# viniciusvidal2/slam-sensor-fusion

Hardware: AMD Instinct MI355X
Metric: scans_per_s_200k_scan_vs_10M_map (higher is better)
Workload: dtype f32 points / f64 accumulation

## Files before the change

### include/slamfusion.h

```cpp
#ifndef SLAMFUSION_H
#define SLAMFUSION_H
#include <stdint.h>

#ifdef __cplusplus
extern "C" {
#endif

#define SF_VERSION 210

typedef enum {
    SF_OK = 0,
    SF_ERR_INVALID = -1,
    SF_ERR_HIP = -2,
    SF_ERR_NOMEM = -3,
    SF_ERR_STATE = -4,
    SF_ERR_OVERFLOW = -5,
    SF_ERR_COMM = -6
} sf_status;

typedef struct sf_ctx sf_ctx;
typedef struct sf_cloud sf_cloud;
typedef struct sf_map sf_map;
typedef struct sf_icp sf_icp;

// ... 252 lines not shown
int sf_icp_fetch_previous(sf_icp *icp, sf_icp_result *out);
int sf_icp_use_graph(sf_icp *icp, int on);
int sf_icp_graph_counts(sf_icp *icp, int64_t *captures, int64_t *launches);
int sf_icp_set_fused(sf_icp *icp, int on);
int sf_icp_fused_count(sf_icp *icp, int64_t *launches);
int sf_icp_fused_redone(sf_icp *icp, int64_t *redone);
int sf_icp_test_inject_barrier_timeout(sf_icp *icp);
#define SF_ORDER_AUTO 0
#define SF_ORDER_AS_GIVEN 1
#define SF_ORDER_CELL 2
int sf_icp_set_query_order(sf_icp *icp, int order);
int sf_icp_set_nn_reuse(sf_icp *icp, int on);
int sf_icp_set_wide_scan_points(sf_icp *icp, int64_t points);
int sf_icp_set_pipeline(sf_icp *icp, int on);
int sf_icp_set_tile_search(sf_icp *icp, int mode);
int sf_icp_tile_info(sf_icp *icp, int64_t out[12]);
int sf_icp_set_freeze(sf_icp *icp, int on);
int sf_icp_set_freeze_params(sf_icp *icp, float guard_scale, float guard_min, float guard_max, int max_tries, int from_launch);
int sf_icp_freeze_stats(sf_icp *icp, int64_t out[5]);
int sf_icp_set_defer_search(sf_icp *icp, int on);
int sf_icp_defer_stats(sf_icp *icp, int64_t out[2]);
int sf_icp_lookup_launch_stats(sf_icp *icp, int64_t out[4]);
int sf_icp_set_neighbour_research(sf_icp *icp, int from_launch);
int sf_icp_neighbour_stats(sf_icp *icp, int64_t out[3]);
int sf_icp_neighbour_gap_stats(sf_icp *icp, int64_t out[4]);
#define SF_ROBUST_NONE 0
#define SF_ROBUST_HUBER 1
#define SF_ROBUST_CAUCHY 2
#define SF_ROBUST_TUKEY 3
#define SF_ROBUST_GM 4
int sf_icp_set_robust_kernel(sf_icp *icp, int kind, double k);

#define SF_COV_EIG_EPS 1e-12
#define SF_COV_FEW_CORR 1
#define SF_COV_SINGULAR 2
#define SF_COV_DEGENERATE_TRANS 4
#define SF_COV_DEGENERATE_ROT 8
typedef struct {
    double info[36];
    double cov[36];
    double sigma2, sigma2_hat, weight_sum;
    double trans_info[3], trans_dir[9];
    double rot_info[3], rot_dir[9];
    int64_t n_corr;
    int32_t flags;
} sf_icp_covariance;
// ... 218 lines not shown
```

### slam_sensor_fusion_amd/api.py

```python
import atexit
import ctypes as C
import math
import os
import weakref

import numpy as np

_HERE = os.path.dirname(os.path.abspath(__file__))
LIB_PATH = os.path.join(_HERE, "lib", "libslamfusion.so")

SF_ICP_REF_CPP, SF_ICP_O3D_P2P, SF_ICP_P2PLANE = 0, 1, 2
SF_VOXEL_PCL, SF_VOXEL_O3D, SF_VOXEL_PCL64 = 0, 1, 2
SF_FLAG_VOXEL_OVERFLOW = 1
SF_ICP_FLAG_FEW_CORR, SF_ICP_FLAG_SINGULAR, SF_ICP_FLAG_SHARD_STALE, SF_ICP_FLAG_BARRIER_TIMEOUT = 1, 2, 4, 8
PROF_NN, PROF_REDUCE, PROF_COLLECTIVE, PROF_SOLVE, PROF_SHARD_BUILD = 0, 1, 2, 3, 4
SF_ERR_COMM = -6
MODES = {"ref_cpp": SF_ICP_REF_CPP, "o3d_p2p": SF_ICP_O3D_P2P, "p2plane": SF_ICP_P2PLANE}
ROBUST_KINDS = {"none": 0, "huber": 1, "cauchy": 2, "tukey": 3, "gm": 4}


class SlamFusionError(RuntimeError):
    pass


# ... 1515 lines not shown
        code = {False: 0, "off": 0, "auto": 1, True: 2, "always": 2}[on]
        _check(self.lib.sf_icp_set_tile_search(self.h, C.c_int(code)))

    def tile_info(self):
        a = (C.c_int64 * 12)()
        _check(self.lib.sf_icp_tile_info(self.h, a))
        return {"on": bool(a[0]), "cells_per_tile": [a[1], a[2], a[3]], "tiles": [a[4], a[5], a[6]], "searched": a[7], "from_lds": a[8], "left_region": a[9],
                "beyond_ring_1": a[10], "tiles_too_dense": a[11]}

    def set_freeze_params(self, guard_scale=8.0, guard_min=2.0e-5, guard_max=3.0e-4, max_tries=3, from_launch=5):
        _check(self.lib.sf_icp_set_freeze_params(self.h, C.c_float(guard_scale), C.c_float(guard_min), C.c_float(guard_max), C.c_int(max_tries), C.c_int(from_launch)))

    def freeze_stats(self):
        a = (C.c_int64 * 5)()
        _check(self.lib.sf_icp_freeze_stats(self.h, a))
        return {"froze": a[0], "thawed": a[1], "failed": a[2], "active_queries": a[3], "frozen_at_end": a[4]}

    def set_defer_search(self, on=True):
        _check(self.lib.sf_icp_set_defer_search(self.h, C.c_int(int(bool(on)))))

    def set_neighbour_research(self, from_launch=2):
        _check(self.lib.sf_icp_set_neighbour_research(self.h, C.c_int(int(from_launch))))

    def neighbour_stats(self):
        a = (C.c_int64 * 3)()
        _check(self.lib.sf_icp_neighbour_stats(self.h, a))
        return {"served": a[0], "not_served": a[1], "waves_searched": a[2]}

    def neighbour_gap_stats(self):
        a = (C.c_int64 * 4)()
        _check(self.lib.sf_icp_neighbour_gap_stats(self.h, a))
        return {"served": a[0], "not_served": a[1], "waves_searched": a[2], "by_gap": a[3]}

    def defer_stats(self):
        a = (C.c_int64 * 2)()
        _check(self.lib.sf_icp_defer_stats(self.h, a))
        return {"deferred_queries": a[0], "capped_waves": a[1]}

    def lookup_launch_stats(self):
        a = (C.c_int64 * 4)()
        _check(self.lib.sf_icp_lookup_launch_stats(self.h, a))
        return {"launches": a[0], "deferred_queries": a[1], "capped_waves": a[2], "first": a[3]}

    def set_query_order(self, order="auto"):
        _check(self.lib.sf_icp_set_query_order(self.h, C.c_int({"auto": 0, "as_given": 1, "cell": 2}[order])))

# ... 689 lines not shown
```

### slam_sensor_fusion_amd/csrc/sf_icp.hip

```cpp
#include "sf_common.hpp"
#include "sf_nn.hpp"
#include "sf_tile.hpp"
#include "sf_order.hpp"
#include "sf_p2p.hpp"
#include "sf_schedule.hpp"
#include "sf_sort.hpp"

#include <cfloat>
#include <cstdlib>
#include <cmath>
#include <vector>
#include <mutex>
#include <string>
#include <type_traits>

namespace {

constexpr int BLK = 256;
constexpr int NREC_P2P = 17;
constexpr int NREC_PLANE = 30;
constexpr int REC_STRIDE = 32;

struct IcpState {
    double T[16];
// ... 1781 lines not shown
        }
    }
#pragma unroll
    for (int h = 0; h < 2; ++h) {
        double v[16];
#pragma unroll
        for (int k = 0; k < 16; ++k) v[k] = 0.0;
#pragma unroll
        for (int u = 0; u < Q; ++u) {
            const PairTerms t = pair_terms<MODE>(P[u]);
            add_half<MODE>(t, h, v);
        }
        const double t0 = wave_reduce_16(v);
        if ((lane & 3) == 0) stage[wv][16 * h + (lane >> 2)] = t0;
    }
    __syncthreads();
    if (threadIdx.x < NREC) {
        const int c = threadIdx.x;
        double *dst = partials + ((size_t)b * nblocks + bx) * REC_STRIDE;
        dst[c] = ((stage[0][c] + stage[1][c]) + stage[2][c]) + stage[3][c];
    }
}

template <int Q>
__global__ __launch_bounds__(BLK, 2) void k_nn_deferred(SfGrid g, SfWindow w, const float *__restrict__ X0x, const float *__restrict__ X0y, const float *__restrict__ X0z,
                                                                   int n, const IcpState *__restrict__ st, float thr, int nblocks, float4 *__restrict__ qcache, int64_t cache_n,
                                                                   uint32_t *__restrict__ stats, DeferBufs df)
{
    constexpr int MODE = 2;
    constexpr int NW = BLK / 64;
    const int r = (int)blockIdx.x, b = (int)blockIdx.y;
    const IcpState *S = st + b;
    if (S->done) return;
    __shared__ sf::WaveNN nn_ws[NW];
    __shared__ double fstage[NW][32];
    __shared__ uint32_t list[BLK * DF_WCAP];
    __shared__ uint32_t wsum[NW];
    __shared__ uint32_t capped;
    const int wv = threadIdx.x >> 6, lane = threadIdx.x & 63;
    if (threadIdx.x == 0) capped = 0u;
    __syncthreads();
    const int my_rows = r < nblocks ? (nblocks - r + FZ_FEW - 1) / FZ_FEW : 0;
    const int nseg = my_rows * NW;
    double acc = 0.0;
    uint32_t n_listed = 0;
    for (int s0 = 0; s0 < nseg; s0 += BLK) {
        const int sg = s0 + (int)threadIdx.x;
        const int bx = r + (sg / NW) * FZ_FEW;
        const size_t seg = ((size_t)b * nblocks + bx) * NW + (sg % NW);
        uint32_t c = sg < nseg ? (uint32_t)df.cnt[seg] : 0u;
        if (c > (uint32_t)DF_WCAP) {
            atomicAdd(&capped, 1u);
            c = 0u;
        }
        uint32_t incl = c;
#pragma unroll
        for (int off = 1; off < 64; off <<= 1) {
            const uint32_t t = __shfl_up(incl, off, 64);
            if (lane >= off) incl += t;
        }
        if (lane == 63) wsum[wv] = incl;
        __syncthreads();
        uint32_t base = 0, total = 0;
#pragma unroll
        for (int ww = 0; ww < NW; ++ww) {
            if (ww < wv) base += wsum[ww];
            total += wsum[ww];
        }
        const uint32_t start = base + incl - c;
        for (uint32_t i = 0; i < c; ++i) list[start + i] = (uint32_t)bx * (uint32_t)(BLK * Q) + (uint32_t)df.ids[seg * DF_WCAP + i];
        __syncthreads();
        n_listed += total;
        for (uint32_t q0 = 0; q0 < total; q0 += BLK) {
            const uint32_t i = q0 + (uint32_t)threadIdx.x;
            if (q0 + (uint32_t)(wv * 64) < total) {
                const int slot = i < total ? (int)list[i] : n;
                const LanePair A1 = nn_pair<MODE, false, false>(g, w, X0x, X0y, X0z, n, b, S, thr, 0.0f, 0.0f, nullptr, qcache, cache_n, slot, n, &nn_ws[wv], stats, nullptr, false);
#pragma unroll
                for (int h = 0; h < 2; ++h) {
                    double v[16];
#pragma unroll
                    for (int k = 0; k < 16; ++k) v[k] = 0.0;
                    const PairTerms t = pair_terms<MODE>(A1);
                    add_half<MODE>(t, h, v);
                    const double t0 = wave_reduce_16(v);
                    if ((lane & 3) == 0) fstage[wv][16 * h + (lane >> 2)] = t0;
                }
            } else if (lane < 32) {
                fstage[wv][lane] = 0.0;
            }
            __syncthreads();
            if (threadIdx.x < 32) acc += ((fstage[0][threadIdx.x] + fstage[1][threadIdx.x]) + fstage[2][threadIdx.x]) + fstage[3][threadIdx.x];
            __syncthreads();
        }
    }
    if (threadIdx.x < REC_STRIDE) df.part[((size_t)b * FZ_FEW + r) * REC_STRIDE + threadIdx.x] = threadIdx.x < NREC_PLANE ? acc : 0.0;
    __syncthreads();
    if (threadIdx.x == 0) {
        if (n_listed) atomicAdd(&df.stat[0], n_listed);
        if (capped) {
// ... 821 lines not shown

void prof_collect(sf_icp *icp)
{
    for (size_t k = 0; k + 1 < icp->ev_used; k += 2) {
        float ms = 0;
        if (hipEventElapsedTime(&ms, icp->ev[k], icp->ev[k + 1]) != hipSuccess) continue;
        const int kind = k / 2 < icp->ev_kind.size() ? icp->ev_kind[k / 2] : SF_PROF_NN;
        if (kind == SF_PROF_NN) { icp->prof_ms += ms; icp->prof_launches += 1; icp->prof_each.push_back(ms); }
        else if (kind > 0 && kind < SF_PROF_KINDS) icp->prof_phase[kind].push_back(ms);
    }
    icp->ev_used = 0;
}

void schedule_describe(sf_icp *icp, int mode, bool whole)
{
    const SrcSet &ss = icp->src();
    sf::Schedule in;
    in.mode = mode; in.K = icp->prm.num_iters; in.qpl = ss.qpl; in.sharded = icp->shard; in.whole = whole; in.reuse = icp->reuse; in.window = icp->map->window.kind;
    in.robust = robust_on(icp, mode); in.fz_from = icp->fz_from; in.defer = icp->defer != 0; in.table = icp->nbr_active; in.nbr_from = icp->nbr_active ? icp->nbr_from : -1;
    in.lk_min = icp->lk_min; in.tile_on = icp->tile_on;
    in.wanted = icp->freeze == 2 || (icp->freeze == 1 && (icp->shard ? icp->own_total : ss.n * ss.batch) >= FREEZE_AUTO_MIN_QUERIES);
    icp->cur().meta.sched = sf::make_schedule(in);
    icp->cur().meta.lk_waves = (int64_t)ss.batch * ss.nblocks_nn * (BLK / 64);
}

int slab_rows(const sf_icp *icp, bool sharded, bool one_per_lane)
{
    if (sharded) return one_per_lane ? icp->own_nblocks * icp->src().qpl : icp->own_nblocks;
    return one_per_lane ? icp->src().nblocks : icp->src().nblocks_nn;
}

uint32_t *nn_stats_slot(sf_icp *icp)
{
    if (!icp->profiling || !icp->nn_stats.p || icp->nn_stats_used >= sf_icp::NN_STATS_CAP) return nullptr;
    return icp->nn_stats.as<uint32_t>() + NN_STATS_PER * NN_STATS_SHARDS * icp->nn_stats_used++;
}

sf_icp::GraphKey graph_key_now(const sf_icp *icp, int mode)
{
    const Lane &ln = icp->cur(); const SrcSet &ss = icp->src();
    sf_icp::GraphKey k;
    k.batch = ss.batch; k.ordered = (int)icp->ordered; k.sched = ln.meta.sched;
    k.n = (mode == SF_ICP_REF_CPP && ss.batch == 1) ? -ss.n_cap : ss.n;
    k.map = (const void *)icp->map;
    k.map_generation = icp->map->generation;
    if (icp->nbr_active) { k.nbr_stamp = icp->map->nbr_stamp; k.nbr = icp->map->nbr.p; }
    k.robust_kind = robust_on(icp, mode) ? icp->robust_kind : SF_ROBUST_NONE; k.robust_k = robust_on(icp, mode) ? icp->robust_k : 0.0;
    k.cov_on = icp->cov_on;
    if (icp->cov_on) { const double cp[5] = {icp->cov_arg.sensor_sigma, icp->cov_arg.thr_t, icp->cov_arg.thr_r, icp->cov_arg.infl_t, icp->cov_arg.infl_r}; std::memcpy(k.cov_prm, cp, sizeof(cp)); }
    k.max_corr = icp->prm.max_corr; k.accept = icp->prm.accept; k.eps = icp->prm.eps;
    k.guard_scale = icp->fz_prm.guard_scale; k.guard_min = icp->fz_prm.guard_min; k.guard_max = icp->fz_prm.guard_max; k.max_tries = icp->fz_prm.max_tries;
    const sf::DevBuf *bufs[] = {&ss.X0, &ss.X0r, &ln.X, &ln.Xq, &ln.qcache, &ln.corr, &ln.state, &ln.partials, &icp->d_box, &ss.d_boxes, &ss.n_dev,
                                &icp->map->pts4, &icp->map->nrm4, &icp->map->cell_start, &icp->map->d_window, &ln.fz_state, &ln.fz_part, &ln.fz_cnt, &ln.fz_ids, &ln.fz_all, &ln.df_cnt, &ln.df_ids, &ln.df_part, &ln.df_stat, &ln.tseg, &ln.tile_stats, &ln.cov_part, &ln.cov_out};
    k.epochs = (uint64_t)ss.plane;
    for (const sf::DevBuf *b : bufs) k.epochs = (k.epochs * 1000003ull + b->epoch) * 1000003ull + (uint64_t)(uintptr_t)b->p;
    return k;
}

SfGrid grid_for(const sf_icp *icp)
{
    SfGrid g = icp->map->grid;
    g.nbr = icp->nbr_active ? icp->map->nbr.as<uint4>() : nullptr;
    g.nbr_from = icp->nbr_from;
    return g;
}

int nbr_prepare(sf_icp *icp, int mode)
{
    sf_map *m = icp->map;
    const SrcSet &ss = icp->src();
    icp->nbr_active = false;
// ... 90 lines not shown
{
    Lane &ln = icp->cur();
    FreezeBufs fb;
    fb.fz = on ? ln.fz_state.as<FreezeState>() : nullptr;
    fb.mom_part = ln.fz_part.as<double>();
    fb.act_cnt = ln.fz_cnt.as<uint32_t>();
    fb.act_ids = ln.fz_ids.as<uint16_t>();
    fb.act_all = ln.fz_all.as<uint32_t>();
    fb.df_part = deferred ? ln.df_part.as<double>() : nullptr;
    return fb;
}

DeferBufs defer_bufs(sf_icp *icp)
{
    Lane &ln = icp->cur();
    DeferBufs d;
    d.cnt = ln.df_cnt.as<uint8_t>();
    d.ids = ln.df_ids.as<uint16_t>();
    d.part = ln.df_part.as<double>();
    d.stat = ln.df_stat.as<uint32_t>();
    return d;
}

void launch_nn_deferred(sf_icp *icp, uint32_t *stats)
{
    Lane &ln = icp->cur(); SrcSet &ss = icp->src();
    sf_map *m = icp->map;
    hipLaunchKernelGGL((k_nn_deferred<SF_WIDE_QPL>), dim3((unsigned)FZ_FEW, (unsigned)ss.batch), dim3(BLK), 0, icp->ctx->stream, grid_for(icp), m->window, queries(icp, 0), queries(icp, 1), queries(icp, 2),
                       (int)ss.n, ln.state.as<IcpState>(), o3d_thr(icp), ss.nblocks_nn, ln.qcache.as<float4>(), icp->cache_n, stats, defer_bufs(icp));
}

void launch_nn_red_df(sf_icp *icp, int attempt_from)
{
    Lane &ln = icp->cur(); SrcSet &ss = icp->src();
    sf_map *m = icp->map;
    const int nb = ss.nblocks_nn;
    const dim3 grid((unsigned)((nb + 7) & ~7), (unsigned)ss.batch), blk(BLK);
    ProfScope ps(icp);
    uint32_t *stats = nn_stats_slot(icp);
    hipLaunchKernelGGL((k_nn_red_df<SF_WIDE_QPL>), grid, blk, 0, icp->ctx->stream, grid_for(icp), m->window, queries(icp, 0), queries(icp, 1), queries(icp, 2), (int)ss.n, ln.state.as<IcpState>(),
                       o3d_thr(icp), ln.partials.as<double>(), nb, ln.qcache.as<float4>(), icp->cache_n, stats, defer_bufs(icp), attempt_from);
    launch_nn_deferred(icp, stats);
}

void launch_nn_red_fz(sf_icp *icp, bool sharded, bool few)
{
    Lane &ln = icp->cur(); SrcSet &ss = icp->src();
    sf_map *m = icp->map;
    const int nb = slab_rows(icp, sharded, false);
    const dim3 grid_full((unsigned)((nb + 7) & ~7), (unsigned)ss.batch), grid_few((unsigned)FZ_FEW, (unsigned)ss.batch), blk(BLK);
    ProfScope ps(icp);
    FzArgs A;
    A.X0x = queries(icp, 0); A.X0y = queries(icp, 1); A.X0z = queries(icp, 2);
    A.n = (int)ss.n;
    A.st = ln.state.as<IcpState>();
    A.thr = o3d_thr(icp); A.xlo = icp->xlo; A.xhi = icp->xhi;
    A.partials = ln.partials.as<double>();
    A.nblocks = nb;
    A.own_off = icp->own_off.as<uint32_t>();
    A.qcache = ln.qcache.as<float4>();
    A.cache_n = icp->cache_n;
    A.stats = nn_stats_slot(icp);
    A.fz = ln.fz_state.as<FreezeState>();
    A.mom_part = ln.fz_part.as<double>();
    A.act_cnt = ln.fz_cnt.as<uint32_t>();
    A.act_ids = ln.fz_ids.as<uint16_t>();
    A.act_all = ln.fz_all.as<uint32_t>();
    hipStream_t s = icp->ctx->stream;
    if (few) with_bools([&](auto S) { hipLaunchKernelGGL((k_nn_red_fz_few<SF_WIDE_QPL, S()>), grid_few, blk, 0, s, grid_for(icp), m->window, A); }, sharded);
    else with_bools([&](auto S) { hipLaunchKernelGGL((k_nn_red_fz<SF_WIDE_QPL, S()>), grid_full, blk, 0, s, grid_for(icp), m->window, A); }, sharded);
}

template <int MODE>
void launch_nn(sf_icp *icp, const sf::LaunchStep &step, bool sharded)
{
    if (step.frozen()) launch_nn_red_fz(icp, sharded, step.nn == sf::NN_FROZEN_FEW);
    else if (step.nn == sf::NN_DEFERRING) launch_nn_red_df(icp, step.attempt_from);
    else if (step.nn == sf::NN_TILE_SEARCH) launch_tile_search<MODE>(icp, step.one_per_lane);
    else launch_nn_red<MODE>(icp, sharded, step.one_per_lane);
}

int step_start_pass(sf_icp *icp, int mode)
{
    Lane &ln = icp->cur(); SrcSet &ss = icp->src();
    icp->fz_step = 0;
    schedule_describe(icp, mode, false);
    if (!ln.meta.sched.fz) return SF_OK;
    SF_TRY(freeze_alloc(icp));
    hipLaunchKernelGGL(k_fz_init, dim3(nblk(ss.batch, 64)), dim3(64), 0, icp->ctx->stream, ln.fz_state.as<FreezeState>(), ss.batch, ln.df_stat.as<uint32_t>());
    return SF_OK;
}

int launch_state_init(sf_icp *icp)
{
    Lane &ln = icp->cur();
    hipStream_t s = icp->ctx->stream;
    const int B = icp->src().batch;
    InitArgs args;
    if (B <= INIT_ARGS_MAX) {
        std::memcpy(args.T, icp->inits.data(), sizeof(double) * 16 * (size_t)B);
// ... 536 lines not shown
{
    SF_CHECK(icp && out, SF_ERR_INVALID, "bad arguments");
    for (int i = 0; i < 12; ++i) out[i] = 0;
    out[0] = icp->tile_on ? 1 : 0;
    if (!icp->tile_on) return SF_OK;
    for (int a = 0; a < 3; ++a) { out[1 + a] = icp->tiles.tc[a]; out[4 + a] = icp->tiles.nt[a]; }
    if (icp->cur().tile_stats.p) {
        SF_HIP(hipSetDevice(icp->ctx->device));
        unsigned long long h[TILE_STATS];
        SF_HIP(hipMemcpyAsync(h, icp->cur().tile_stats.p, sizeof(h), hipMemcpyDeviceToHost, icp->ctx->stream));
        SF_HIP(hipStreamSynchronize(icp->ctx->stream));
        for (int i = 0; i < 5; ++i) out[7 + i] = (int64_t)h[i];
    }
    return SF_OK;
}

extern "C" int sf_icp_set_defer_search(sf_icp *icp, int on)
{
    SF_CHECK(icp, SF_ERR_INVALID, "icp is NULL");
    icp->defer = on != 0;
    return SF_OK;
}

extern "C" int sf_icp_set_neighbour_research(sf_icp *icp, int from_launch)
{
    SF_CHECK(icp, SF_ERR_INVALID, "icp is NULL");
    SF_CHECK(from_launch != 0, SF_ERR_INVALID, "from_launch must be at least 1 (the first launch has no cached neighbours), or negative for off");
    icp->nbr_from = from_launch < 0 ? -1 : from_launch;
    icp->lk_min = 0;
    return SF_OK;
}

namespace {
int neighbour_stats(sf_icp *icp, int64_t out[4])
{
    SF_CHECK(icp && out, SF_ERR_INVALID, "bad arguments");
    SF_CHECK(icp->profiling && icp->nn_stats.p, SF_ERR_STATE, "the neighbour statistics are counted in profiled runs (sf_icp_profile_enable)");
    SF_CHECK(icp->nn_stats_used < sf_icp::NN_STATS_CAP, SF_ERR_STATE, "the profiling counters are full (%lld launches since sf_icp_profile_enable): enable profiling again to reset them", (long long)sf_icp::NN_STATS_CAP);
    SF_HIP(hipStreamSynchronize(icp->ctx->stream));
    out[0] = out[1] = out[2] = out[3] = 0;
    const int64_t first = icp->nbr_stats_first, used = icp->nn_stats_used;
    if (used <= first) return SF_OK;
    const size_t per = (size_t)NN_STATS_PER * NN_STATS_SHARDS;
    std::vector<uint32_t> st(per * (size_t)(used - first), 0u);
    SF_HIP(hipMemcpy(st.data(), icp->nn_stats.as<uint32_t>() + per * (size_t)first, sizeof(uint32_t) * st.size(), hipMemcpyDeviceToHost));
    for (size_t i = 0; i < st.size(); i += NN_STATS_PER) { out[0] += st[i + 2]; out[1] += st[i + 3]; out[2] += st[i + 1]; out[3] += st[i + 4]; }
    return SF_OK;
}
}

extern "C" int sf_icp_neighbour_stats(sf_icp *icp, int64_t out[3])
{
// ... 25 lines not shown
    out[0] = out[1] = out[2] = 0;
    out[3] = -1;
    const sf::Schedule &sched = icp->cur().meta.sched;
    if (sched.lookup_launches() <= 0) return SF_OK;
    int64_t df[2];
    SF_TRY(sf_icp_defer_stats(icp, df));
    out[0] = sched.lookup_launches();
    out[1] = df[0];
    out[2] = df[1];
    out[3] = sched.lookup_first;
    return SF_OK;
}

extern "C" int sf_icp_set_freeze(sf_icp *icp, int on)
{
    SF_CHECK(icp, SF_ERR_INVALID, "icp is NULL");
    SF_CHECK(on >= 0 && on <= 2, SF_ERR_INVALID, "sf_icp_set_freeze: 0 (off), 1 (auto) or 2 (always)");
    icp->freeze = on;
    return SF_OK;
}

namespace {
constexpr int FZ_FROM_DEFAULT = 5, FZ_PROBE_EVERY = 32;
void freeze_learn_schedule(sf_icp *icp)
{
    const sf::Schedule &sched = icp->cur().meta.sched;
    if (!icp->fz_from_auto || icp->last_fused || icp->shard || icp->last_mode != SF_ICP_P2PLANE) return;
    const int K = sched.K;
    if (++icp->fz_fetches >= FZ_PROBE_EVERY) { icp->fz_fetches = 0; icp->fz_from = FZ_FROM_DEFAULT; icp->lk_min = 0; return; }
    if (!sched.fz) return;
    if (sched.lookup_launches() > 0 && icp->cur().df_stat.p) {
        uint32_t h[2 + DF_STAT_LAUNCHES];
        if (hipMemcpy(h, icp->cur().df_stat.p, sizeof(h), hipMemcpyDeviceToHost) == hipSuccess) {
            for (int k = sched.lookup_first; k < sched.fz_from && k < DF_STAT_LAUNCHES - 1; ++k)
                if ((int64_t)h[2 + k] * 8 > icp->cur().meta.lk_waves) icp->lk_min = std::max(icp->lk_min, k + 1);
        }
    }
    int latest = -1, never = 0;
    for (int b = 0; b < icp->src().batch; ++b) {
        const IcpState &S = icp->h_state[(size_t)b];
        if (S.froze_launch >= 0) latest = std::max(latest, S.froze_launch);
        else if (S.iterations >= K) never += 1;
    }
    if (latest < 0) icp->fz_from = std::max(FZ_FROM_DEFAULT, K);
    else if (never * 4 <= icp->src().batch) icp->fz_from = std::min(std::max(FZ_FROM_DEFAULT, latest), std::max(FZ_FROM_DEFAULT, K - 2));
}
}

extern "C" int sf_icp_set_robust_kernel(sf_icp *icp, int kind, double k)
{
    SF_CHECK(icp, SF_ERR_INVALID, "icp is NULL");
    SF_CHECK(kind >= SF_ROBUST_NONE && kind <= SF_ROBUST_GM, SF_ERR_INVALID, "unknown robust kernel %d", kind);
    SF_CHECK(kind == SF_ROBUST_NONE || (std::isfinite(k) && k > 0.0), SF_ERR_INVALID, "the robust kernel's scale must be finite and > 0 (got %g)", k);
    icp->robust_kind = kind;
    icp->robust_k = kind == SF_ROBUST_NONE ? 0.0 : k;
    return SF_OK;
}

// ... 211 lines not shown
    if (icp->profiling) prof_collect(icp);
    SF_TRY(check_barrier_flags(icp, nb));
    for (int b = 0; b < nb; ++b)
        fill_result(icp, described ? ln.meta.mode : icp->last_mode, icp->h_state[(size_t)b], described ? &ln.meta.inits[(size_t)b * 16] : &icp->inits[(size_t)b * 16], out + b);
    if (nb == ss.batch) freeze_learn_schedule(icp);
    return SF_OK;
}

extern "C" int sf_icp_fetch_previous(sf_icp *icp, sf_icp_result *out)
{
    SF_CHECK(icp && out, SF_ERR_INVALID, "bad arguments");
    Lane &pl = icp->prev();
    const sf_icp::LaneMeta &M = pl.meta;
    SF_CHECK(icp->prev_ok && M.valid && M.batch > 0, SF_ERR_STATE,
             "no earlier alignment to fetch: the latest alignment did not run beside the one before it (fetched in between, pipeline off, single launch) or it was fetched already");
    SF_CHECK(pl.used && pl.done && pl.stream && pl.state.p, SF_ERR_STATE, "the other lane holds no alignment");
    SF_HIP(hipSetDevice(icp->ctx->device));
    SF_HIP(hipEventSynchronize(pl.done));
    icp->h_prev.resize((size_t)M.batch);
    SF_HIP(hipMemcpyAsync(icp->h_prev.data(), pl.state.p, sizeof(IcpState) * (size_t)M.batch, hipMemcpyDeviceToHost, pl.stream));
    SF_HIP(hipStreamSynchronize(pl.stream));
    for (int b = 0; b < M.batch; ++b) fill_result(icp, M.mode, icp->h_prev[(size_t)b], &M.inits[(size_t)b * 16], out + b);
    icp->prev_ok = false;
    return SF_OK;
}

extern "C" int sf_icp_set_covariance(sf_icp *icp, int on, double sensor_sigma)
{
    SF_CHECK(icp, SF_ERR_INVALID, "icp is NULL");
    SF_CHECK(std::isfinite(sensor_sigma) && sensor_sigma >= 0.0, SF_ERR_INVALID, "sensor_sigma must be finite and >= 0 (0: the estimated residual variance)");
    icp->cov_on = on != 0;
    icp->cov_arg.sensor_sigma = sensor_sigma;
    return SF_OK;
}

extern "C" int sf_icp_set_degeneracy_thresholds(sf_icp *icp, double trans, double rot, double inflate_trans_var, double inflate_rot_var)
{
    SF_CHECK(icp, SF_ERR_INVALID, "icp is NULL");
    const double v[4] = {trans, rot, inflate_trans_var, inflate_rot_var};
    for (double x : v) SF_CHECK(std::isfinite(x) && x >= 0.0, SF_ERR_INVALID, "thresholds and inflations must be finite and >= 0");
    icp->cov_arg.thr_t = trans; icp->cov_arg.thr_r = rot;
    icp->cov_arg.infl_t = inflate_trans_var; icp->cov_arg.infl_r = inflate_rot_var;
    return SF_OK;
}

extern "C" int sf_icp_fetch_covariance(sf_icp *icp, sf_icp_covariance *out)
// ... 525 lines not shown
```

### slam_sensor_fusion_amd/csrc/sf_icp_object.hpp

```cpp

struct sf_icp {
    sf_ctx *ctx = nullptr;
    IcpParams prm{};
    int debug = 0;
    int64_t cache_n = 0;
    bool reuse = true;
    int order = SF_ORDER_AUTO;
    bool ordered = false;
    std::vector<double> inits;
    double *h_inits = nullptr;
    size_t h_inits_cap = 0;
    hipEvent_t inits_ev = nullptr;
    bool inits_ev_pending = false;
    sf_map *map = nullptr;
    sf_map *own_map = nullptr;
    sf_cloud *own_cloud = nullptr;
    sf::DevBuf xchg_own;
    void *xchg = nullptr;
    int64_t xchg_bytes = 0;
    int64_t wide_from = WIDE_SCAN_POINTS;
    bool wide_auto = true;
    std::vector<IcpState> h_state;
    bool shard = false;
    float xlo = 0, xhi = 0;
    sf::DevBuf own_idx, own_blk, own_count, own_off, own_keep;
    std::vector<uint32_t> h_own;
    int64_t own_total = 0;
    float own_margin = 1.0f;
    int own_nblocks = 1;
    sf::DevBuf d_box;
    int last_mode = 0;
    bool fused = true;
    bool last_fused = false;
    sf::DevBuf bar;
    int fused_limit[4] = {-1, -1, -1, -1};
    double fused_share = 0.0;
    int64_t fused_redone = 0;
    bool inject_timeout = false;
    int64_t fused_launches = 0;
    IcpState *h_pin = nullptr;
    size_t h_pin_cap = 0;
    bool use_graph = false;
    int64_t graph_captures = 0, graph_replays = 0;
    struct GraphKey {
        int batch = -1, ordered = -1, robust_kind = -1, cov_on = -1;
        sf::Schedule sched;
        int64_t n = -1;
        const void *map = nullptr;
        uint64_t map_generation = 0, epochs = 0;
        uint64_t nbr_stamp = 0;
        const void *nbr = nullptr;
        float max_corr = 0, accept = 0, eps = 0, guard_scale = 0, guard_min = 0, guard_max = 0;
        int max_tries = 0;
        double robust_k = 0;
        double cov_prm[5] = {0, 0, 0, 0, 0};
        bool operator==(const GraphKey &o) const
        {
            return batch == o.batch && ordered == o.ordered && sched == o.sched && n == o.n && map == o.map && map_generation == o.map_generation && epochs == o.epochs &&
                   nbr_stamp == o.nbr_stamp && nbr == o.nbr && max_corr == o.max_corr && accept == o.accept && eps == o.eps &&
                   guard_scale == o.guard_scale && guard_min == o.guard_min && guard_max == o.guard_max && max_tries == o.max_tries &&
                   robust_kind == o.robust_kind && robust_k == o.robust_k && cov_on == o.cov_on && std::memcmp(cov_prm, o.cov_prm, sizeof(cov_prm)) == 0;
        }
    };
    struct LaneMeta {
        bool valid = false;
        bool cov = false;
        int batch = 0, mode = 0;
        std::vector<double> inits;
        int src_set = 0;
        uint64_t src_version = 0;
        sf::Schedule sched;
        int64_t lk_waves = 0;
    };
    struct Lane {
        sf::DevBuf X;
        sf::DevBuf qcache;
        sf::DevBuf Xq, qkeys, qkeys2, qidx, qidx2;
        sf::DevBuf corr;
        sf::DevBuf state, d_inits, partials;
        sf::DevBuf fz_state, fz_part, fz_cnt, fz_ids, fz_all;
        sf::DevBuf df_cnt, df_ids, df_part, df_stat;
        sf::DevBuf qtkey, tseg, tile_stats;
        sf::DevBuf cov_part, cov_out;
        hipGraphExec_t graph_exec = nullptr;
        GraphKey graph_key;
        std::vector<double> inits_uploaded;
        uint32_t d_inits_epoch = 0xffffffffu;
        hipStream_t stream = nullptr;
        hipEvent_t done = nullptr;
        bool used = false;
        hipEvent_t started = nullptr;
        bool started_rec = false;
        LaneMeta meta;
    } lanes[2];
    int lane = 0;
// ... 37 lines not shown
    uint64_t src_version = 0, mark_src_version = 0, mark_map_generation = 0;
    const void *mark_map = nullptr;
    SfWindow mark_window{};
    bool profiling = false;
    std::vector<hipEvent_t> ev;
    size_t ev_used = 0;
    int64_t prof_launches = 0;
    double prof_ms = 0;
    std::vector<float> prof_each;
    std::vector<int> ev_kind;
    std::vector<float> prof_phase[SF_PROF_KINDS];
    sf::DevBuf nn_stats;
    int freeze = 1;
    FreezeParams fz_prm{8.0f, 2.0e-5f, 3.0e-4f, 3};
    int fz_from = 5;
    bool fz_from_auto = true;
    int fz_fetches = 0;
    int fz_step = 0;
    int nbr_from = SF_NBR_FROM;
    bool nbr_active = false;
    int64_t nbr_stats_first = 0;
    uint64_t mark_nbr_stamp = 0;
    int defer = 1;
    int lk_min = 0;
    int64_t nn_stats_used = 0;
    static constexpr int64_t NN_STATS_CAP = 1024;
    int robust_kind = SF_ROBUST_NONE;
    double robust_k = 0.0;
    int cov_on = 0;
    CovArg cov_arg{0.0, 0.0, 0.0, 0.0, 0.0};
    bool prev_cov_ok = false;
    int tile_mode = 0;
    bool tile_on = false;
    sf::SfTiles tiles{};
};

namespace {

using Lane = sf_icp::Lane;
using SrcSet = sf_icp::SrcSet;
float *soa(sf::DevBuf &b, int64_t total, int axis) { return b.as<float>() + (size_t)axis * (size_t)total; }
const float *queries(sf_icp *icp, int axis)
{
    Lane &ln = icp->cur(); SrcSet &ss = icp->src();
    if (icp->shard) return soa(ln.Xq, icp->own_total, axis);
    return soa(icp->ordered ? ln.Xq : ss.X0, ss.plane, axis);
// ... 31 lines not shown
```

### slam_sensor_fusion_amd/csrc/sf_schedule.hpp

```cpp
#pragma once
#include "slamfusion.h"

#ifndef SF_WIDE_QPL
#define SF_WIDE_QPL 2
#endif

namespace sf {

constexpr int VERIFY_FROM_SEARCH = 4;

struct Schedule {
    int mode = 0, K = 0, qpl = 1;
    int sharded = 0, whole = 0;
    int reuse = 0, window = 0;
    int robust = 0, wanted = 0;
    int fz_from = 0, defer = 0;
    int table = 0, nbr_from = 0;
    int lk_min = 0, tile_on = 0;
    int fz = 0, lookup_first = 0, defer_first = 0;
    bool operator==(const Schedule &o) const
    {
        return mode == o.mode && K == o.K && qpl == o.qpl && sharded == o.sharded && whole == o.whole && reuse == o.reuse && window == o.window && robust == o.robust &&
               wanted == o.wanted && fz_from == o.fz_from && defer == o.defer && table == o.table && nbr_from == o.nbr_from && lk_min == o.lk_min && tile_on == o.tile_on &&
               fz == o.fz && lookup_first == o.lookup_first && defer_first == o.defer_first;
    }
    bool deferring() const { return defer_first < fz_from; }
    int lookup_launches() const { return fz_from - lookup_first; }
};

enum NnForm { NN_SEARCH = 0, NN_TILE_SEARCH = 1, NN_DEFERRING = 2, NN_FREEZE = 3, NN_FROZEN_FEW = 4 };
struct LaunchStep {
    int nn = NN_SEARCH;
    int one_per_lane = 0;
    int solve_takes_freeze_state = 0;
    int ask_freeze = 0;
    int deferred_rows = 0;
    int attempt_from = 0;
    bool frozen() const { return nn == NN_FREEZE || nn == NN_FROZEN_FEW; }
};

inline Schedule make_schedule(Schedule s)
{
    s.fz = s.mode == SF_ICP_P2PLANE && s.wanted && !s.robust && s.reuse && s.qpl == SF_WIDE_QPL && s.window == 0 && s.K > s.fz_from + 1 && s.fz_from >= VERIFY_FROM_SEARCH;
    const bool df = s.fz && s.defer && !s.sharded;
    const int lk = s.nbr_from > s.lk_min ? s.nbr_from : s.lk_min;
    s.lookup_first = df && s.table && s.nbr_from >= 1 && lk < s.fz_from ? lk : s.fz_from;
    const int last = s.fz_from - 1 >= VERIFY_FROM_SEARCH ? s.fz_from - 1 : s.fz_from;
    s.defer_first = !df ? s.fz_from : s.lookup_first < last ? s.lookup_first : last;
    return s;
}

inline int launches(int mode, int K) { return mode == SF_ICP_O3D_P2P ? K + 1 : K; }
inline int launches(const Schedule &s) { return launches(s.mode, s.K); }

inline LaunchStep step_of(const Schedule &s, int k)
{
    LaunchStep st;
    const bool df = k >= s.defer_first && k < s.fz_from;
    st.one_per_lane = s.mode == SF_ICP_P2PLANE && s.qpl > 1 && k < VERIFY_FROM_SEARCH && !df;
    if (s.fz && k == s.fz_from) st.nn = NN_FREEZE;
    else if (s.fz && k > s.fz_from) st.nn = NN_FROZEN_FEW;
    else if (df) st.nn = NN_DEFERRING;
    else if (s.whole && s.tile_on && (!s.reuse || k < VERIFY_FROM_SEARCH)) st.nn = NN_TILE_SEARCH;
    st.solve_takes_freeze_state = s.fz && k + 1 >= s.fz_from;
    st.ask_freeze = st.solve_takes_freeze_state && k + 2 < s.K;
    st.deferred_rows = df;
    st.attempt_from = s.lookup_first < s.fz_from ? s.lookup_first : VERIFY_FROM_SEARCH;
    return st;
}

}
```

Measured before the change: 23430.

## Add lean lookup-only NN kernel that defers capped waves to deferred kernel

Adds k_nn_lookup, a lighter kernel with higher occupancy bounds that only tries the reuse certificate and neighbour table for each query and never runs an inline grid search. Waves with too many failing queries are marked capped and recomputed wholesale in k_nn_deferred, which gains a redo path that scans every query of those waves. A host-side learner uses df_stat counts to fall back to the old in-place kernel per launch when capped waves are frequent, and the new settings are added to the graph cache key. The aim is to cut register pressure and divergence in the lookup launches, at the cost of extra deferred work when many waves get capped.

```diff
diff --git a/include/slamfusion.h b/include/slamfusion.h
--- a/include/slamfusion.h
+++ b/include/slamfusion.h
@@ -298,6 +298,7 @@
 int sf_icp_defer_stats(sf_icp *icp, int64_t out[2]);
 int sf_icp_lookup_launch_stats(sf_icp *icp, int64_t out[4]);
 int sf_icp_set_neighbour_research(sf_icp *icp, int from_launch);
+int sf_icp_set_lookup_kernel(sf_icp *icp, int on);
 int sf_icp_neighbour_stats(sf_icp *icp, int64_t out[3]);
 int sf_icp_neighbour_gap_stats(sf_icp *icp, int64_t out[4]);
 #define SF_ROBUST_NONE 0
diff --git a/slam_sensor_fusion_amd/api.py b/slam_sensor_fusion_amd/api.py
--- a/slam_sensor_fusion_amd/api.py
+++ b/slam_sensor_fusion_amd/api.py
@@ -1561,6 +1561,9 @@
     def set_neighbour_research(self, from_launch=2):
         _check(self.lib.sf_icp_set_neighbour_research(self.h, C.c_int(int(from_launch))))
 
+    def set_lookup_kernel(self, on=True):
+        _check(self.lib.sf_icp_set_lookup_kernel(self.h, C.c_int(int(bool(on)))))
+
     def neighbour_stats(self):
         a = (C.c_int64 * 3)()
         _check(self.lib.sf_icp_neighbour_stats(self.h, a))
diff --git a/slam_sensor_fusion_amd/csrc/sf_icp.hip b/slam_sensor_fusion_amd/csrc/sf_icp.hip
--- a/slam_sensor_fusion_amd/csrc/sf_icp.hip
+++ b/slam_sensor_fusion_amd/csrc/sf_icp.hip
@@ -1827,10 +1827,107 @@
     }
 }
 
+#ifndef SF_LOOKUP_WAVES
+#define SF_LOOKUP_WAVES 6
+#endif
+template <int Q>
+__global__ __launch_bounds__(BLK, SF_LOOKUP_WAVES) void k_nn_lookup(SfGrid g, SfWindow w, const float *__restrict__ X0x, const float *__restrict__ X0y, const float *__restrict__ X0z,
+                                                                    int n, const IcpState *__restrict__ st, float thr, double *__restrict__ partials, int nblocks,
+                                                                    float4 *__restrict__ qcache, int64_t cache_n, uint32_t *__restrict__ stats, DeferBufs df, int attempt_from)
+{
+    constexpr int MODE = 2;
+    constexpr int NREC = NREC_PLANE;
+    const int L = blockIdx.y * gridDim.x + blockIdx.x;
+    const int kk = L >> 3;
+    const int b = kk % (int)gridDim.y;
+    const int bx = (L & 7) * ((int)gridDim.x >> 3) + kk / (int)gridDim.y;
+    if (bx >= nblocks) return;
+    const IcpState *S = st + b;
+    if (S->done) return;
+    __shared__ double stage[BLK / 64][32];
+    const int wv = threadIdx.x >> 6, lane = threadIdx.x & 63;
+    const size_t seg = ((size_t)b * nblocks + bx) * (BLK / 64) + wv;
+    LanePair P[Q];
+    bool need[Q];
+#pragma unroll
+    for (int u = 0; u < Q; ++u) {
+        need[u] = false;
+        P[u].sx = P[u].sy = P[u].sz = 0.0;
+        P[u].px = P[u].py = P[u].pz = 0.0f;
+        P[u].tn = make_float4(0.f, 0.f, 0.f, 0.f);
+        P[u].ok = false;
+    }
+    const bool attempted = qcache != nullptr && S->cache_live != 0 && S->n_research >= attempt_from;
+    bool fast = false;
+    uint32_t listed = 0;
+    if (attempted) {
+        const float m_now = (float)S->motion;
+#pragma unroll
+        for (int u = 0; u < Q; ++u) {
+            const int slot = bx * (BLK * Q) + u * BLK + (int)threadIdx.x;
+            const QueryIn q = query_in<MODE, false>(X0x, X0y, X0z, n, b, S, 0.0f, 0.0f, nullptr, qcache, cache_n, true, slot, n);
+            sf::NNHit hit, seed;
+            float4 tn;
+            need[u] = reuse_certificate(q.valid, q.qx, q.qy, q.qz, thr, m_now, q.e, q.c1, q.c2, hit, tn, seed);
+            if (g.nbr != nullptr && S->n_research >= g.nbr_from) {
+                const bool tried = need[u] && seed.j >= 0;
+                int served = 0;
+                if (tried) {
+                    served = table_serve<MODE>(g, q, thr, m_now, seed, qcache, cache_n, hit, tn);
+                    need[u] = served == 0;
+                }
+                if (stats) table_count(stats, tried, served);
+            }
+            P[u] = make_pair(q, hit, tn);
+        }
+        uint32_t failing = 0;
+#pragma unroll
+        for (int u = 0; u < Q; ++u) failing += (uint32_t)__popcll(__ballot(need[u]));
+        fast = failing <= (uint32_t)DF_WCAP;
+        listed = fast ? failing : (uint32_t)DF_CAPPED;
+    } else {
+        listed = (uint32_t)DF_CAPPED;
+    }
+    if (lane == 0) df.cnt[seg] = (uint8_t)listed;
+    if (fast && listed != 0u) {
+        uint32_t before = 0;
+#pragma unroll
+        for (int u = 0; u < Q; ++u) {
+            const unsigned long long bal = __ballot(need[u]);
+            const uint32_t rank = (uint32_t)__builtin_amdgcn_mbcnt_hi((uint32_t)(bal >> 32), __builtin_amdgcn_mbcnt_lo((uint32_t)bal, 0u));
+            if (need[u]) df.ids[seg * DF_WCAP + before + rank] = (uint16_t)(u * BLK + (int)threadIdx.x);
+            before += (uint32_t)__popcll(bal);
+        }
+    }
+    if (!fast) {
+#pragma unroll
+        for (int u = 0; u < Q; ++u) P[u].ok = false;
+    }
+#pragma unroll
+    for (int h = 0; h < 2; ++h) {
+        double v[16];
+#pragma unroll
+        for (int k = 0; k < 16; ++k) v[k] = 0.0;
+#pragma unroll
+        for (int u = 0; u < Q; ++u) {
+            const PairTerms t = pair_terms<MODE>(P[u]);
+            add_half<MODE>(t, h, v);
+        }
+        const double t0 = wave_reduce_16(v);
+        if ((lane & 3) == 0) stage[wv][16 * h + (lane >> 2)] = t0;
+    }
+    __syncthreads();
+    if (threadIdx.x < NREC) {
+        const int c = threadIdx.x;
+        double *dst = partials + ((size_t)b * nblocks + bx) * REC_STRIDE;
+        dst[c] = ((stage[0][c] + stage[1][c]) + stage[2][c]) + stage[3][c];
+    }
+}
+
 template <int Q>
 __global__ __launch_bounds__(BLK, 2) void k_nn_deferred(SfGrid g, SfWindow w, const float *__restrict__ X0x, const float *__restrict__ X0y, const float *__restrict__ X0z,
                                                                    int n, const IcpState *__restrict__ st, float thr, int nblocks, float4 *__restrict__ qcache, int64_t cache_n,
-                                                                   uint32_t *__restrict__ stats, DeferBufs df)
+                                                                   uint32_t *__restrict__ stats, DeferBufs df, int redo_capped)
 {
     constexpr int MODE = 2;
     constexpr int NW = BLK / 64;
@@ -1840,6 +1937,7 @@
     __shared__ sf::WaveNN nn_ws[NW];
     __shared__ double fstage[NW][32];
     __shared__ uint32_t list[BLK * DF_WCAP];
+    __shared__ uint16_t cseg[BLK];
     __shared__ uint32_t wsum[NW];
     __shared__ uint32_t capped;
     const int wv = threadIdx.x >> 6, lane = threadIdx.x & 63;
@@ -1854,11 +1952,13 @@
         const int bx = r + (sg / NW) * FZ_FEW;
         const size_t seg = ((size_t)b * nblocks + bx) * NW + (sg % NW);
         uint32_t c = sg < nseg ? (uint32_t)df.cnt[seg] : 0u;
+        uint32_t cap = 0u;
         if (c > (uint32_t)DF_WCAP) {
             atomicAdd(&capped, 1u);
             c = 0u;
-        }
-        uint32_t incl = c;
+            cap = redo_capped ? 1u : 0u;
+        }
+        uint32_t incl = c | (cap << 16);
 #pragma unroll
         for (int off = 1; off < 64; off <<= 1) {
             const uint32_t t = __shfl_up(incl, off, 64);
@@ -1866,21 +1966,37 @@
         }
         if (lane == 63) wsum[wv] = incl;
         __syncthreads();
-        uint32_t base = 0, total = 0;
+        uint32_t base = 0, both = 0;
 #pragma unroll
         for (int ww = 0; ww < NW; ++ww) {
             if (ww < wv) base += wsum[ww];
-            total += wsum[ww];
-        }
-        const uint32_t start = base + incl - c;
+            both += wsum[ww];
+        }
+        const uint32_t total = both & 0xffffu, ncap = both >> 16;
+        const uint32_t start = ((base + incl) & 0xffffu) - c;
         for (uint32_t i = 0; i < c; ++i) list[start + i] = (uint32_t)bx * (uint32_t)(BLK * Q) + (uint32_t)df.ids[seg * DF_WCAP + i];
+        if (cap) cseg[((base + incl) >> 16) - 1u] = (uint16_t)threadIdx.x;
         __syncthreads();
         n_listed += total;
-        for (uint32_t q0 = 0; q0 < total; q0 += BLK) {
-            const uint32_t i = q0 + (uint32_t)threadIdx.x;
-            if (q0 + (uint32_t)(wv * 64) < total) {
-                const int slot = i < total ? (int)list[i] : n;
-                const LanePair A1 = nn_pair<MODE, false, false>(g, w, X0x, X0y, X0z, n, b, S, thr, 0.0f, 0.0f, nullptr, qcache, cache_n, slot, n, &nn_ws[wv], stats, nullptr, false);
+        const uint32_t r_listed = (total + (uint32_t)BLK - 1u) / (uint32_t)BLK, r_all = r_listed + (ncap * (uint32_t)Q + (uint32_t)NW - 1u) / (uint32_t)NW;
+        for (uint32_t t = 0; t < r_all; ++t) {
+            const bool redo = t >= r_listed;
+            int slot = n;
+            bool active;
+            if (!redo) {
+                const uint32_t i = t * (uint32_t)BLK + (uint32_t)threadIdx.x;
+                active = t * (uint32_t)BLK + (uint32_t)(wv * 64) < total;
+                if (i < total) slot = (int)list[i];
+            } else {
+                const uint32_t j = (t - r_listed) * (uint32_t)NW + (uint32_t)wv;
+                active = j < ncap * (uint32_t)Q;
+                if (active) {
+                    const int sgc = s0 + (int)cseg[j / (uint32_t)Q];
+                    slot = (r + (sgc / NW) * FZ_FEW) * (BLK * Q) + (int)(j % (uint32_t)Q) * BLK + (sgc % NW) * 64 + lane;
+                }
+            }
+            if (active) {
+                const LanePair A1 = nn_pair<MODE, false, false>(g, w, X0x, X0y, X0z, n, b, S, thr, 0.0f, 0.0f, nullptr, qcache, cache_n, slot, n, &nn_ws[wv], stats, nullptr, redo);
 #pragma unroll
                 for (int h = 0; h < 2; ++h) {
                     double v[16];
@@ -2748,6 +2864,8 @@
     in.wanted = icp->freeze == 2 || (icp->freeze == 1 && (icp->shard ? icp->own_total : ss.n * ss.batch) >= FREEZE_AUTO_MIN_QUERIES);
     icp->cur().meta.sched = sf::make_schedule(in);
     icp->cur().meta.lk_waves = (int64_t)ss.batch * ss.nblocks_nn * (BLK / 64);
+    icp->cur().meta.lookup_kernel = icp->lookup_kernel;
+    icp->cur().meta.lk_inplace = icp->fz_from_auto ? icp->lk_inplace : 0u;
 }
 
 int slab_rows(const sf_icp *icp, bool sharded, bool one_per_lane)
@@ -2773,6 +2891,7 @@
     if (icp->nbr_active) { k.nbr_stamp = icp->map->nbr_stamp; k.nbr = icp->map->nbr.p; }
     k.robust_kind = robust_on(icp, mode) ? icp->robust_kind : SF_ROBUST_NONE; k.robust_k = robust_on(icp, mode) ? icp->robust_k : 0.0;
     k.cov_on = icp->cov_on;
+    k.lookup_kernel = ln.meta.lookup_kernel; k.lk_inplace = ln.meta.lk_inplace;
     if (icp->cov_on) { const double cp[5] = {icp->cov_arg.sensor_sigma, icp->cov_arg.thr_t, icp->cov_arg.thr_r, icp->cov_arg.infl_t, icp->cov_arg.infl_r}; std::memcpy(k.cov_prm, cp, sizeof(cp)); }
     k.max_corr = icp->prm.max_corr; k.accept = icp->prm.accept; k.eps = icp->prm.eps;
     k.guard_scale = icp->fz_prm.guard_scale; k.guard_min = icp->fz_prm.guard_min; k.guard_max = icp->fz_prm.guard_max; k.max_tries = icp->fz_prm.max_tries;
@@ -2909,15 +3028,15 @@
     return d;
 }
 
-void launch_nn_deferred(sf_icp *icp, uint32_t *stats)
+void launch_nn_deferred(sf_icp *icp, uint32_t *stats, bool redo_capped)
 {
     Lane &ln = icp->cur(); SrcSet &ss = icp->src();
     sf_map *m = icp->map;
     hipLaunchKernelGGL((k_nn_deferred<SF_WIDE_QPL>), dim3((unsigned)FZ_FEW, (unsigned)ss.batch), dim3(BLK), 0, icp->ctx->stream, grid_for(icp), m->window, queries(icp, 0), queries(icp, 1), queries(icp, 2),
-                       (int)ss.n, ln.state.as<IcpState>(), o3d_thr(icp), ss.nblocks_nn, ln.qcache.as<float4>(), icp->cache_n, stats, defer_bufs(icp));
-}
-
-void launch_nn_red_df(sf_icp *icp, int attempt_from)
+                       (int)ss.n, ln.state.as<IcpState>(), o3d_thr(icp), ss.nblocks_nn, ln.qcache.as<float4>(), icp->cache_n, stats, defer_bufs(icp), (int)redo_capped);
+}
+
+void launch_nn_red_df(sf_icp *icp, int attempt_from, int index)
 {
     Lane &ln = icp->cur(); SrcSet &ss = icp->src();
     sf_map *m = icp->map;
@@ -2925,9 +3044,14 @@
     const dim3 grid((unsigned)((nb + 7) & ~7), (unsigned)ss.batch), blk(BLK);
     ProfScope ps(icp);
     uint32_t *stats = nn_stats_slot(icp);
-    hipLaunchKernelGGL((k_nn_red_df<SF_WIDE_QPL>), grid, blk, 0, icp->ctx->stream, grid_for(icp), m->window, queries(icp, 0), queries(icp, 1), queries(icp, 2), (int)ss.n, ln.state.as<IcpState>(),
-                       o3d_thr(icp), ln.partials.as<double>(), nb, ln.qcache.as<float4>(), icp->cache_n, stats, defer_bufs(icp), attempt_from);
-    launch_nn_deferred(icp, stats);
+    const bool lookup = ln.meta.lookup_kernel && ln.meta.sched.lookup_launches() > 0 && !((ln.meta.lk_inplace >> std::min(index, 31)) & 1u);
+    if (lookup)
+        hipLaunchKernelGGL((k_nn_lookup<SF_WIDE_QPL>), grid, blk, 0, icp->ctx->stream, grid_for(icp), m->window, queries(icp, 0), queries(icp, 1), queries(icp, 2), (int)ss.n, ln.state.as<IcpState>(),
+                           o3d_thr(icp), ln.partials.as<double>(), nb, ln.qcache.as<float4>(), icp->cache_n, stats, defer_bufs(icp), attempt_from);
+    else
+        hipLaunchKernelGGL((k_nn_red_df<SF_WIDE_QPL>), grid, blk, 0, icp->ctx->stream, grid_for(icp), m->window, queries(icp, 0), queries(icp, 1), queries(icp, 2), (int)ss.n, ln.state.as<IcpState>(),
+                           o3d_thr(icp), ln.partials.as<double>(), nb, ln.qcache.as<float4>(), icp->cache_n, stats, defer_bufs(icp), attempt_from);
+    launch_nn_deferred(icp, stats, lookup);
 }
 
 void launch_nn_red_fz(sf_icp *icp, bool sharded, bool few)
@@ -2962,7 +3086,7 @@
 void launch_nn(sf_icp *icp, const sf::LaunchStep &step, bool sharded)
 {
     if (step.frozen()) launch_nn_red_fz(icp, sharded, step.nn == sf::NN_FROZEN_FEW);
-    else if (step.nn == sf::NN_DEFERRING) launch_nn_red_df(icp, step.attempt_from);
+    else if (step.nn == sf::NN_DEFERRING) launch_nn_red_df(icp, step.attempt_from, step.index);
     else if (step.nn == sf::NN_TILE_SEARCH) launch_tile_search<MODE>(icp, step.one_per_lane);
     else launch_nn_red<MODE>(icp, sharded, step.one_per_lane);
 }
@@ -3545,12 +3669,20 @@
     return SF_OK;
 }
 
+extern "C" int sf_icp_set_lookup_kernel(sf_icp *icp, int on)
+{
+    SF_CHECK(icp, SF_ERR_INVALID, "icp is NULL");
+    icp->lookup_kernel = on != 0;
+    return SF_OK;
+}
+
 extern "C" int sf_icp_set_neighbour_research(sf_icp *icp, int from_launch)
 {
     SF_CHECK(icp, SF_ERR_INVALID, "icp is NULL");
     SF_CHECK(from_launch != 0, SF_ERR_INVALID, "from_launch must be at least 1 (the first launch has no cached neighbours), or negative for off");
     icp->nbr_from = from_launch < 0 ? -1 : from_launch;
     icp->lk_min = 0;
+    icp->lk_inplace = 0u;
     return SF_OK;
 }
 
@@ -3622,6 +3754,18 @@
 
 namespace {
 constexpr int FZ_FROM_DEFAULT = 5, FZ_PROBE_EVERY = 32;
+#ifndef SF_LK_CAPPED_ONE_IN
+#define SF_LK_CAPPED_ONE_IN 1024
+#endif
+void lookup_learn_kernel(sf_icp *icp, const sf_icp::LaneMeta &M, const uint32_t *h)
+{
+    for (int k = M.sched.lookup_first; k < M.sched.fz_from && k < DF_STAT_LAUNCHES - 1; ++k) {
+        const uint32_t bit = 1u << k;
+        if ((int64_t)h[2 + k] * SF_LK_CAPPED_ONE_IN > M.lk_waves) icp->lk_inplace |= bit;
+        else icp->lk_inplace &= ~bit;
+    }
+}
+
 void freeze_learn_schedule(sf_icp *icp)
 {
     const sf::Schedule &sched = icp->cur().meta.sched;
@@ -3634,6 +3778,7 @@
         if (hipMemcpy(h, icp->cur().df_stat.p, sizeof(h), hipMemcpyDeviceToHost) == hipSuccess) {
             for (int k = sched.lookup_first; k < sched.fz_from && k < DF_STAT_LAUNCHES - 1; ++k)
                 if ((int64_t)h[2 + k] * 8 > icp->cur().meta.lk_waves) icp->lk_min = std::max(icp->lk_min, k + 1);
+            lookup_learn_kernel(icp, icp->cur().meta, h);
         }
     }
     int latest = -1, never = 0;
@@ -3891,6 +4036,12 @@
     SF_HIP(hipStreamSynchronize(pl.stream));
     for (int b = 0; b < M.batch; ++b) fill_result(icp, M.mode, icp->h_prev[(size_t)b], &M.inits[(size_t)b * 16], out + b);
     icp->prev_ok = false;
+    if (icp->fz_from_auto && !icp->shard && M.mode == SF_ICP_P2PLANE && M.sched.fz && M.sched.lookup_launches() > 0 && pl.df_stat.p) {
+        uint32_t h[2 + DF_STAT_LAUNCHES];
+        SF_HIP(hipMemcpyAsync(h, pl.df_stat.p, sizeof(h), hipMemcpyDeviceToHost, pl.stream));
+        SF_HIP(hipStreamSynchronize(pl.stream));
+        lookup_learn_kernel(icp, M, h);
+    }
     return SF_OK;
 }
 
diff --git a/slam_sensor_fusion_amd/csrc/sf_icp_object.hpp b/slam_sensor_fusion_amd/csrc/sf_icp_object.hpp
--- a/slam_sensor_fusion_amd/csrc/sf_icp_object.hpp
+++ b/slam_sensor_fusion_amd/csrc/sf_icp_object.hpp
@@ -43,7 +43,8 @@
     bool use_graph = false;
     int64_t graph_captures = 0, graph_replays = 0;
     struct GraphKey {
-        int batch = -1, ordered = -1, robust_kind = -1, cov_on = -1;
+        int batch = -1, ordered = -1, robust_kind = -1, cov_on = -1, lookup_kernel = -1;
+        uint32_t lk_inplace = 0;
         sf::Schedule sched;
         int64_t n = -1;
         const void *map = nullptr;
@@ -59,7 +60,7 @@
             return batch == o.batch && ordered == o.ordered && sched == o.sched && n == o.n && map == o.map && map_generation == o.map_generation && epochs == o.epochs &&
                    nbr_stamp == o.nbr_stamp && nbr == o.nbr && max_corr == o.max_corr && accept == o.accept && eps == o.eps &&
                    guard_scale == o.guard_scale && guard_min == o.guard_min && guard_max == o.guard_max && max_tries == o.max_tries &&
-                   robust_kind == o.robust_kind && robust_k == o.robust_k && cov_on == o.cov_on && std::memcmp(cov_prm, o.cov_prm, sizeof(cov_prm)) == 0;
+                   robust_kind == o.robust_kind && robust_k == o.robust_k && cov_on == o.cov_on && lookup_kernel == o.lookup_kernel && lk_inplace == o.lk_inplace && std::memcmp(cov_prm, o.cov_prm, sizeof(cov_prm)) == 0;
         }
     };
     struct LaneMeta {
@@ -71,6 +72,8 @@
         uint64_t src_version = 0;
         sf::Schedule sched;
         int64_t lk_waves = 0;
+        int lookup_kernel = 0;
+        uint32_t lk_inplace = 0;
     };
     struct Lane {
         sf::DevBuf X;
@@ -154,6 +157,8 @@
     int64_t nbr_stats_first = 0;
     uint64_t mark_nbr_stamp = 0;
     int defer = 1;
+    int lookup_kernel = 1;
+    uint32_t lk_inplace = 0u;
     int lk_min = 0;
     int64_t nn_stats_used = 0;
     static constexpr int64_t NN_STATS_CAP = 1024;
diff --git a/slam_sensor_fusion_amd/csrc/sf_schedule.hpp b/slam_sensor_fusion_amd/csrc/sf_schedule.hpp
--- a/slam_sensor_fusion_amd/csrc/sf_schedule.hpp
+++ b/slam_sensor_fusion_amd/csrc/sf_schedule.hpp
@@ -30,6 +30,7 @@
 
 enum NnForm { NN_SEARCH = 0, NN_TILE_SEARCH = 1, NN_DEFERRING = 2, NN_FREEZE = 3, NN_FROZEN_FEW = 4 };
 struct LaunchStep {
+    int index = 0;
     int nn = NN_SEARCH;
     int one_per_lane = 0;
     int solve_takes_freeze_state = 0;
@@ -56,6 +57,7 @@
 inline LaunchStep step_of(const Schedule &s, int k)
 {
     LaunchStep st;
+    st.index = k;
     const bool df = k >= s.defer_first && k < s.fz_from;
     st.one_per_lane = s.mode == SF_ICP_P2PLANE && s.qpl > 1 && k < VERIFY_FROM_SEARCH && !df;
     if (s.fz && k == s.fz_from) st.nn = NN_FREEZE;
```

Result: slower. 23020 (-1.8%).
